# dist1ll/pomcpp

Hardware: AMD Instinct MI355X
Metric: env_steps_per_sec (higher is better)
Workload: dtype int32

## Files before the change

### pomcpp_amd/csrc/pom_step_body.h

```cpp
#ifndef POM_STEP_BODY_H_
#define POM_STEP_BODY_H_

#include "pom_packed.h"

#if defined(__clang__)
#define POM_NOUNROLL _Pragma("nounroll")
#else
#define POM_NOUNROLL
#endif
#define POM_N 11
#define POM_Q 20
#define POM_STACK_DEPTH 21

#if defined(POM_DIAG) && defined(__HIP_DEVICE_COMPILE__)
#define POM_STAMP(L, k)                                   \
    do {                                                  \
        const long long now_ = (long long)clock64();      \
        (L).t_acc[k] += now_ - (L).t_last;                \
        (L).t_last = now_;                                \
    } while (0)
#else
#define POM_STAMP(L, k) ((void)0)
#endif
#if defined(POM_TRUNC)
// ... 44 lines not shown
POM_HD int pb_pos(int b) { return b & 0xFF; }
POM_HD int pb_id(int b) { return (b >> 8) & 0xF; }
POM_HD int pb_strength(int b) { return (b >> 12) & 0xF; }
POM_HD int pb_time(int b) { return (b >> 16) & 0xF; }
POM_HD int pb_dir(int b) { return (b >> 20) & 0xF; }
POM_HD int pb_set(int b, uint32_t mask, uint32_t v) { return (int)(((uint32_t)b & ~mask) + v); }

#if defined(__HIP_DEVICE_COMPILE__)
#define POM_IN_VGPR(x) asm("" : "+v"(x))
#else
#define POM_IN_VGPR(x) ((void)0)
#endif
POM_HD int sel4(int i, const int v[4])
{
    int v0 = v[0], v1 = v[1], v2 = v[2], v3 = v[3];
    POM_IN_VGPR(v0);
    POM_IN_VGPR(v1);
    POM_IN_VGPR(v2);
    POM_IN_VGPR(v3);
    const int lo = (i & 1) ? v1 : v0, hi = (i & 1) ? v3 : v2;
    return (i & 2) ? hi : lo;
}
POM_HD uint32_t pick4(int i, const uint32_t v[4])
{
    const uint32_t lo = (i & 1) ? v[1] : v[0], hi = (i & 1) ? v[3] : v[2];
    return (i & 2) ? hi : lo;
}
POM_HD void put4(int i, int v[4], int x)
{
    v[0] = i == 0 ? x : v[0];
    v[1] = i == 1 ? x : v[1];
    v[2] = i == 2 ? x : v[2];
    v[3] = i == 3 ? x : v[3];
}
POM_HD int ag_x(int a0) { return a0 & 0xF; }
POM_HD int ag_y(int a0) { return (a0 >> 4) & 0xF; }
POM_HD int ag_pos(int a0) { return a0 & 0xFF; }
POM_HD int ag_dead(int a0) { return (a0 >> 17) & 1; }
POM_HD int ag_kick(int a0) { return (a0 >> 16) & 1; }
POM_HD int ag_setpos(int a0, int x, int y) { return (a0 & ~0xFF) | x | (y << 4); }
POM_HD int ag_bombcount(int a0) { return pom_sext8((uint32_t)a0 >> 8); }
POM_HD int ag_bombcount_add(int a0, int d) { return (a0 & ~0xFF00) | (int)(((uint32_t)a0 + ((uint32_t)d << 8)) & 0xFF00u); }
POM_HD int ag_max_bombs(int a1) { return pom_sext16((uint32_t)a1); }
POM_HD int ag_strength(int a1) { return (a1 >> 16) & 0xFF; }
POM_HD int ag_strength_inc(int a1) { return ag_strength(a1) == 0xFF ? a1 : a1 + (1 << 16); }

POM_HD int wrap20(int p)
{
    const unsigned u = (unsigned)p, w = u - (unsigned)POM_Q;
    return (int)(u < w ? u : w);
}
POM_HD uint32_t pom_zero_bytes(uint32_t x)
{
    return ~(((x & 0x7F7F7F7Fu) + 0x7F7F7F7Fu) | x | 0x7F7F7F7Fu);
}
POM_HD uint32_t pom_byte_x4(uint32_t b)
{
#if defined(__HIP_DEVICE_COMPILE__)
    return __builtin_amdgcn_perm(b, b, 0u);
#else
    return b * 0x01010101u;
#endif
}
template <int K>
POM_HD uint32_t pom_gather_bytes(uint32_t w0, uint32_t w1, uint32_t w2, uint32_t w3)
{
#if defined(__HIP_DEVICE_COMPILE__)
    const uint32_t lo = __builtin_amdgcn_perm(w1, w0, 0x0C0C0400u + K * 0x0101u);
    const uint32_t hi = __builtin_amdgcn_perm(w3, w2, 0x0C0C0400u + K * 0x0101u);
    return __builtin_amdgcn_perm(hi, lo, 0x05040100u);
#else
    return ((w0 >> (8 * K)) & 0xFFu) | (((w1 >> (8 * K)) & 0xFFu) << 8) | (((w2 >> (8 * K)) & 0xFFu) << 16) |
           (((w3 >> (8 * K)) & 0xFFu) << 24);
#endif
}
POM_HD int div11(int c)
{
#if defined(__HIP_DEVICE_COMPILE__)
    return __mul24(c, 373) >> 12;
#else
    return c / POM_N;
#endif
}
POM_HD int oob(int x, int y)
{
    const unsigned ux = (unsigned)x, uy = (unsigned)y;
    return (ux > uy ? ux : uy) >= (unsigned)POM_N;
}

POM_HD int mv_dx(int m) { return (int)((0x55555615u >> (2 * m)) & 3u) - 1; }
POM_HD int mv_dy(int m) { return (int)((0x55555561u >> (2 * m)) & 3u) - 1; }

template <class A>
struct PomStepper {
    A& a;
    PomLane& L;
    uint32_t oldp_ = 0;
    int irregular_ = 0;
    int folded_ = 0;
    uint32_t occ_[4] = {0u, 0u, 0u, 0u};
    int occ_valid_ = 0, occ_keep_ = 0;
    POM_HD PomStepper(A& a_, PomLane& l_) : a(a_), L(l_) {}

    POM_HD int bomb_at(int i) const { return a.bomb(wrap20(L.bIdx + i)); }
    POM_HD void set_bomb_at(int i, int v) { a.set_bomb(wrap20(L.bIdx + i), v); }

    POM_HD int bomb_index(int pos) const
    {
        int r = 99;
        POM_NOUNROLL
        for (int i = a.sub(); i < L.bCnt; i += A::G) {
            if (pb_pos(bomb_at(i)) == pos) {
                r = i;
                break;
            }
        }
        r = a.gmin(r);
        return r == 99 ? -1 : r;
    }
    POM_HD void put_bomb_at(int i, int v) { a.put_bomb(wrap20(L.bIdx + i), v); }
    POM_HD int bomb_index_alone(int pos) const
    {
        POM_NOUNROLL
        for (int i = 0; i < L.bCnt; i += 4) {
            const int b0 = bomb_at(i), b1 = bomb_at(i + 1), b2 = bomb_at(i + 2), b3 = bomb_at(i + 3);
            int r = -1;
            r = ((int)(i + 3 < L.bCnt) & (int)(pb_pos(b3) == pos)) ? i + 3 : r;
            r = ((int)(i + 2 < L.bCnt) & (int)(pb_pos(b2) == pos)) ? i + 2 : r;
            r = ((int)(i + 1 < L.bCnt) & (int)(pb_pos(b1) == pos)) ? i + 1 : r;
            r = pb_pos(b0) == pos ? i : r;
            if (r >= 0) return r;
        }
        return -1;
    }

    POM_HD int get_agent(int x, int y) const
    {
        const int want = x | (y << 4);
        int r = -1;
#pragma unroll
        for (int i = 3; i >= 0; i--)
            r = ((!ag_dead(L.a0[i])) & (int)(ag_pos(L.a0[i]) == want)) ? i : r;
        return r;
    }

    POM_HD void kill(int id)
    {
        if (id >= POM_AGENT_COUNT) {
            L.ub |= POM_UB_BAD_INDEX;
            return;
        }
        int v = sel4(id, L.a0);
        if (!ag_dead(v)) {
            put4(id, L.a0, v | POM_AG_DEAD);
            L.alive--;
        }
    }

    POM_HD void owner_bombcount_dec(int b)
    {
        int id = pb_id(b);
        if (id >= POM_AGENT_COUNT) {
            L.ub |= POM_UB_BAD_INDEX;
            return;
        }
        put4(id, L.a0, ag_bombcount_add(sel4(id, L.a0), -1));
    }

    POM_HD void remove_at(int at)
    {
        POM_NOUNROLL
        for (int i = at + 1 + a.sub(); i < L.bCnt; i += A::G) {
            const int v = bomb_at(i);
            put_bomb_at(i - 1, v);
        }
        a.sync();
        if (folded_) {
            const int w = bomb_at(L.bCnt - 1);
            set_bomb_at(L.bCnt - 1, (w & (1 << 24)) ? (w & ~(1 << 24)) : (int)((uint32_t)w + (1u << 16)));
        }
        L.bCnt--;
    }

    enum { REM_TOP = 62, REM_NONE = 63 };

    POM_HD int owner_strength(int b)
    {
        const int owner = pb_id(b);
        if (owner < POM_AGENT_COUNT) return ag_strength(a.ag1(owner));
        L.ub |= POM_UB_BAD_INDEX;
        return 0;
    }

    POM_HD void flame_prologue(int x, int y, int strength, int e )
    {
        int slot = L.fIdx + L.fCnt;
        if (__builtin_expect(slot >= 2 * POM_Q, 0)) {
            POM_NOUNROLL
            while (slot >= POM_Q) slot -= POM_Q;
        } else {
            slot = wrap20(slot);
        }
        a.set_flame(slot, x | (y << 8) | (POM_FLAME_LIFETIME << 16) | ((strength & 0xFF) << 24));
        if (__builtin_expect(L.fCnt >= 255, 0)) L.ub |= POM_UB_FLAME_QUEUE_RANGE;
        else L.fCnt++;
        const int c = y * POM_N + x;
        if (pc_is_agent(e)) kill(pc_agent_id(e));
        a.set_cell(c, POM_C_FLAME + c);
    }
    POM_HD void flame_prologue(int x, int y, int strength) { flame_prologue(x, y, strength, a.cell(y * POM_N + x)); }

    POM_HD void explode_epilogue(int rem)
    {
        if (rem == REM_TOP) {
            owner_bombcount_dec(bomb_at(0));
            L.bIdx = wrap20(L.bIdx + 1);
            L.bCnt--;
        } else if (rem != REM_NONE) {
            owner_bombcount_dec(bomb_at(rem));
            remove_at(rem);
        }
    }

    POM_HD static int ray_step(int dir)
    {
        return (int)(int8_t)(0xF50BFF01u >> (8 * dir));
    }
    POM_HD static int ray_cell(int c0, int dir, int i)
    {
#if defined(__HIP_DEVICE_COMPILE__)
        return c0 + __mul24(i, ray_step(dir));
#else
        return c0 + i * ray_step(dir);
#endif
    }
    POM_HD static int ray_room(int x, int y, int s, int dir)
    {
        const unsigned rooms = (unsigned)(POM_N - 1 - x) | ((unsigned)x << 4) | ((unsigned)(POM_N - 1 - y) << 8) | ((unsigned)y << 12);
        const int room = (int)((rooms >> (4 * dir)) & 0xFu);
        return room < s ? room : s;
    }

    POM_HD void kill_set(int victims)
    {
#pragma unroll
        for (int j = 0; j < 4; j++) {
            const int hit = (victims >> j) & 1 & !ag_dead(L.a0[j]);
            L.a0[j] |= hit << 17;
            L.alive -= hit;
        }
    }

    POM_HD void explode(int x, int y, int strength, int rem, int top_word = -1)
    {
        int s = strength < 0 ? 0 : strength > POM_N ? POM_N : strength;
        POM_STAMP(L, POM_PH_TICK_BOMBS);
        if (s > 2) {
            explode_long(x, y, strength, rem);
            return;
        }
        {
            const int c0 = y * POM_N + x;
            const int e0 = a.cell(c0);
            int chains = 0, victims = 0;
            int chain_key = 0;
            uint32_t lens = 0;
            uint32_t ends = 0;
            POM_NOUNROLL
            for (int r = a.sub(); r < 4; r += A::G) {
                const int lim = ray_room(x, y, s, r);
                const int on1 = lim >= 1, on2 = lim >= 2;
                const int c1 = ray_cell(c0, r, on1);
                const int e1 = a.cell(c1);
                const int ag1 = pc_is_agent(e1);
                int q1 = 0;
                if (on1 & ((int)(e1 == POM_C_BOMB) | ag1)) {
                    const int cy = div11(c1);
                    q1 = bomb_index_alone((c1 - cy * POM_N) | (cy << 4)) >= 0;
                }
                const int took1 = on1 & !q1 & (int)(e1 != POM_C_RIGID);
                const int wood1 = took1 & pc_is_wood(e1);
                int len = took1, vict = (took1 & ag1) << (pc_agent_id(e1) & 3), flag = wood1 ? pc_wood_flag(e1) : 0;
                if (q1) {
                    chains = 1;
                    chain_key = (1 << 12) | ag1 | ((pc_agent_id(e1) & 3) << 1);
                }
                if (took1 & !wood1 & on2) {
                    const int c2 = ray_cell(c0, r, 2);
                    const int e2 = a.cell(c2);
                    const int ag2 = pc_is_agent(e2);
                    int q2 = 0;
                    if ((int)(e2 == POM_C_BOMB) | ag2) {
                        const int cy = div11(c2);
                        q2 = bomb_index_alone((c2 - cy * POM_N) | (cy << 4)) >= 0;
                    }
                    const int took2 = (int)(q2 == 0) & (int)(e2 != POM_C_RIGID);
                    len += took2;
                    vict |= (took2 & ag2) << (pc_agent_id(e2) & 3);
                    flag = (took2 & pc_is_wood(e2)) ? pc_wood_flag(e2) : flag;
                    if (q2) {
                        chains = 1;
                        chain_key = (2 << 12) | ag2 | ((pc_agent_id(e2) & 3) << 1);
                    }
                }
                victims |= vict;
                ends |= (uint32_t)flag << (2 * r);
                lens |= (uint32_t)len << (4 * r);
            }
            if (__builtin_expect(!a.gor(chains), 1)) {
                flame_prologue(x, y, strength, e0);
                const int killed = a.gor(victims);
                if (killed) kill_set(killed);
                POM_NOUNROLL
                for (int r = a.sub(); r < 4; r += A::G) {
                    const int len = (lens >> (4 * r)) & 0xF, f = (int)((ends >> (2 * r)) & 3u);
                    if (len >= 1) a.put_cell(ray_cell(c0, r, 1), pc_flame_code(c0, r, 1, len == 1 ? f : 0));
                    if (len >= 2) a.put_cell(ray_cell(c0, r, 2), pc_flame_code(c0, r, 2, f));
                }
                a.sync();
                if (rem == REM_TOP && top_word != -1) {
                    owner_bombcount_dec(top_word);
                    L.bIdx = wrap20(L.bIdx + 1);
                    L.bCnt--;
                } else {
                    explode_epilogue(rem);
                }
                return;
            }
            if (A::G == 4) {
                const int r = a.sub();
                explode_long(x, y, strength, rem, 1, (int)((lens >> (4 * r)) & 0xF), (int)((ends >> (2 * r)) & 3u), victims, chain_key, e0);
                return;
            }
        }
        explode_long(x, y, strength, rem);
    }

    POM_HD void bomb_cells(uint32_t occ[4]) const
    {
        occ[0] = occ[1] = occ[2] = occ[3] = 0u;
        if (A::G == 1) {
            POM_NOUNROLL
            for (int k = 0; k < L.bCnt; k++) {
                const int b = bomb_at(k);
                const int idx = pb_y(b) * POM_N + pb_x(b);
// ... 39 lines not shown
        int r = 99;
#pragma unroll
        for (int q = NS - 1; q >= 0; q--) {
            const int k = a.sub() + q * A::G;
            r = (k < L.bCnt && pb_pos(w[q]) == pos) ? k : r;
        }
        r = a.gmin(r);
        return r == 99 ? -1 : r;
    }

    POM_HD void scan_ray(int c0, int r, int start, int lim, const uint32_t occ[4], int& len, int& ends, int& wood, int& vict, int& chain,
                         int& info)
    {
        constexpr int W = 4;
        len = start - 1;
        ends = wood = vict = chain = info = 0;
        const uint32_t H = 0x80808080u;
        POM_NOUNROLL
        for (int i0 = start; i0 <= lim; i0 += W) {
            uint32_t d = 0;
#pragma unroll
            for (int q = 0; q < W; q++)
                d |= (uint32_t)a.cell(ray_cell(c0, r, i0 + q <= lim ? i0 + q : lim)) << (8 * q);
            const int n = lim - i0 + 1;
            const uint32_t onray = n >= W ? H : H >> (8 * (W - n));
            const uint32_t l = d & 0x7F7F7F7Fu, lo = ~d;
            const uint32_t ge1 = l + 0x7F7F7F7Fu, ge2 = l + 0x7E7E7E7Eu, ge3 = l + 0x7D7D7D7Du, ge6 = l + 0x7A7A7A7Au, ge11 = l + 0x75757575u,
                           ge15 = l + 0x71717171u;
            const uint32_t rigid = ge1 & ~ge2 & lo, bombc = ge2 & ~ge3 & lo, woodc = ge6 & ~ge11 & lo & onray, agentc = ge11 & ~ge15 & lo & H;
            const uint32_t fixed = ((rigid | woodc) & onray & H) | (~onray & H);
            const uint32_t fixed_low = fixed & (0u - fixed);
            uint32_t cand = (bombc | agentc) & H & (fixed_low - 1u);
            uint32_t chain_at = 0u;
            POM_NOUNROLL
            while (cand) {
                const int q = __builtin_ctz(cand) >> 3;
                if (cell_in(occ, ray_cell(c0, r, i0 + q))) {
                    chain_at = cand & (0u - cand);
                    break;
                }
                cand &= cand - 1u;
            }
            const uint32_t stop = fixed | chain_at;
            const uint32_t at = stop & (0u - stop), below = at - 1u;
            const int before = __builtin_popcount(below & H);
            const int on_wood = (at & woodc) != 0u;
            len = i0 - 1 + before + on_wood;
            uint32_t dead = agentc & below;
            POM_NOUNROLL
            while (dead) {
                const int q = __builtin_ctz(dead) >> 3;
                dead &= dead - 1u;
                vict |= 1 << pc_agent_id((int)((d >> (8 * q)) & 0xFFu));
            }
            if (at) {
                const int e = (int)((d >> (8 * before)) & 0xFFu);
                if (on_wood) {
                    ends = pc_wood_flag(e);
                    wood = 1;
                }
                if (at & chain_at) {
                    chain = i0 + before;
                    info = pc_is_agent(e) | ((pc_agent_id(e) & 3) << 1);
                }
                break;
            }
        }
    }

    POM_HD void explode_long(int x, int y, int strength, int rem, int seen = 0, int seen_len = 0, int seen_ends = 0, int seen_vict = 0,
                             int seen_chain = 0, int seen_origin = 0)
    {
        int s = strength < 0 ? 0 : strength > POM_N ? POM_N : strength;
        POM_STAMP(L, POM_PH_TICK_BOMBS);
        if (seen) flame_prologue(x, y, strength, seen_origin);
        else flame_prologue(x, y, strength);
        int dir = 0, i = 1, sp = 0;
        constexpr int NR = 4 / A::G;
        uint32_t (&occ)[4] = occ_;
        if (!occ_valid_) bomb_cells(occ);
        occ_valid_ = occ_keep_;
        POM_NOUNROLL
        for (;;) {
            const int c0 = y * POM_N + x;
            int first = 0x7FFFFFFF;
            int rstar, jq = -1;
            if (A::G == 1) {
                POM_NOUNROLL
                for (int r = dir; r < 4 && first == 0x7FFFFFFF; r++) {
                    const int rs1 = r == dir ? i : 1;
                    int len1, ends1, wood1, vict1, chain1, info1;
                    scan_ray(c0, r, rs1, ray_room(x, y, s, r), occ, len1, ends1, wood1, vict1, chain1, info1);
                    if (chain1) {
                        const int c = ray_cell(c0, r, chain1);
                        const int cy = div11(c);
                        jq = bomb_index((c - cy * POM_N) | (cy << 4));
                        if (jq < 0) {
                            const uint32_t m = ~(1u << (c & 31));
                            const int w = c >> 5;
                            occ[0] &= w == 0 ? m : ~0u; occ[1] &= w == 1 ? m : ~0u; occ[2] &= w == 2 ? m : ~0u; occ[3] &= w == 3 ? m : ~0u;
                            r--;
                            continue;
                        }
                        first = (r << 16) | (chain1 << 12) | info1;
                    }
                    POM_NOUNROLL
                    for (int d = rs1; d <= len1; d++)
                        a.put_cell(ray_cell(c0, r, d), pc_flame_code(c0, r, d, (wood1 && d == len1) ? ends1 : 0));
                    kill_set(vict1);
                }
                rstar = first == 0x7FFFFFFF ? 4 : first >> 16;
            } else {
            int rs[NR], rlen[NR], rends[NR], rwood[NR], rvict[NR];
#pragma unroll
            for (int q = 0; q < NR; q++) {
                const int r = a.sub() + q * A::G;
                rs[q] = r == dir ? i : 1;
                int chain = 0, info = 0;
                rlen[q] = rs[q] - 1;
                rends[q] = rwood[q] = rvict[q] = 0;
                if (seen) {
                    rlen[q] = seen_len;
                    rends[q] = seen_ends;
                    rwood[q] = 1;
                    rvict[q] = seen_vict;
                    chain = seen_chain >> 12;
                    info = seen_chain & 0xFFF;
                } else if (r >= dir) scan_ray(c0, r, rs[q], ray_room(x, y, s, r), occ, rlen[q], rends[q], rwood[q], rvict[q], chain, info);
                const int key = (r << 16) | (chain << 12) | info;
                first = (chain != 0 && key < first) ? key : first;
            }
            first = a.gmin(first);
            seen = 0;
            rstar = first == 0x7FFFFFFF ? 4 : first >> 16;
            if (rstar < 4) {
                const int c = ray_cell(c0, rstar, (first >> 12) & 0xF);
                const int cy = div11(c);
                jq = bomb_index_wide((c - cy * POM_N) | (cy << 4));
                if (jq < 0) {
                    const uint32_t m = ~(1u << (c & 31));
                    const int w = c >> 5;
                    occ[0] &= w == 0 ? m : ~0u; occ[1] &= w == 1 ? m : ~0u; occ[2] &= w == 2 ? m : ~0u; occ[3] &= w == 3 ? m : ~0u;
                    continue;
                }
            }
            POM_STAMP(L, POM_PH_X_SCAN);
            int victims = 0;
#pragma unroll
            for (int q = 0; q < NR; q++) {
                const int r = a.sub() + q * A::G;
                if (r >= dir && r <= rstar) {
                    victims |= rvict[q];
                    POM_NOUNROLL
                    for (int d = rs[q]; d <= rlen[q]; d++)
                        a.put_cell(ray_cell(c0, r, d), pc_flame_code(c0, r, d, (rwood[q] && d == rlen[q]) ? rends[q] : 0));
                }
            }
            {
                const int killed = a.gor(victims);
                if (killed) kill_set(killed);
            }
            }
            POM_STAMP(L, POM_PH_X_COMMIT);
            if (rstar == 4) {
                explode_epilogue(rem);
                POM_STAMP(L, POM_PH_X_EPILOGUE);
                if (sp == 0) return;
                sp--;
                const int fr = a.frame(sp);
                x = fr & 0xF; y = (fr >> 4) & 0xF; s = (fr >> 8) & 0xF;
                dir = (fr >> 12) & 7; i = (fr >> 15) & 0xF; rem = (fr >> 19) & 63;
                const int pc0 = y * POM_N + x;
                const int c = ray_cell(pc0, dir, i);
                const int e = a.cell(c);
                int go_on = 0;
                if (e != POM_C_RIGID) {
                    const int was_wood = pc_is_wood(e);
                    a.set_cell(c, pc_flame_code(pc0, dir, i, was_wood ? pc_wood_flag(e) : 0));
                    go_on = !was_wood;
                }
                if (go_on) i++;
                else { dir++; i = 1; }
                continue;
            }
            const int d = (first >> 12) & 0xF;
            if (first & 1) kill((first >> 1) & 3);
            if (sp >= POM_STACK_DEPTH) {
                L.ub |= POM_UB_BAD_INDEX;
                return;
            }
            a.set_frame(sp, x | (y << 4) | (s << 8) | (rstar << 12) | (d << 15) | (rem << 19));
            sp++;
            const int st2 = owner_strength(bomb_at(jq));
            const int c = ray_cell(c0, rstar, d);
            y = div11(c);
            x = c - y * POM_N;
            rem = jq;
            flame_prologue(x, y, st2);
            s = st2 < 0 ? 0 : st2 > POM_N ? POM_N : st2;
            dir = 0;
            i = 1;
            POM_STAMP(L, POM_PH_X_NEST);
        }
    }

    POM_HD void flames_dec(int& top, int& n)
    {
        top = 0;
        n = L.fCnt;
        if (L.fCnt <= 0) return;
        int p = L.fIdx + a.sub();
        p = wrap20(p);
        int held_any = 0;
        POM_NOUNROLL
        for (int i = a.sub(); i < L.fCnt; i += A::G) {
            const int f = a.flame(p);
            const int held = (f & 0xFF0000) == 0x800000;
            const int nf = held ? f : (f & ~0xFF0000) | ((f - 0x10000) & 0xFF0000);
            held_any |= held;
            a.put_flame(p, nf);
            if (p == L.fIdx) top = nf;
            p = wrap20(p + A::G);
        }
        const int v = a.gor(top | (held_any << 7));
        top = v & ~0x80;
        if (v & 0x80) L.ub |= POM_UB_FLAME_QUEUE_RANGE;
    }
    POM_HD void flame_pops(int top, int n)
    {
        POM_NOUNROLL
        for (int k = 0; k < n; k++) {
            const int f = k == 0 ? top : a.flame(L.fIdx);
            if (((f >> 16) & 0xFF) != 0) break;
            const int x = f & 0xFF, y = (f >> 8) & 0xFF;
            int s = (f >> 24) & 0xFF;
            s = s > POM_N ? POM_N : s;
            if (!oob(x, y)) {
                const int c0 = y * POM_N + x;
                if (a.cell(c0) == POM_C_FLAME + c0) a.set_cell(c0, POM_C_PASSAGE);
                POM_NOUNROLL
                for (int r = a.sub(); r < 4; r += A::G) {
                    const int lim = ray_room(x, y, s, r);
                    {
                        const int c = ray_cell(c0, r, lim >= 1);
                        const int to = pc_flame_pops_to(a.cell(c), c0, r, 1);
                        if ((int)(lim >= 1) & (int)(to >= 0)) a.put_cell(c, to);
                    }
                    POM_NOUNROLL
                    for (int i = 2; i <= lim; i++) {
                        const int c = ray_cell(c0, r, i);
                        const int to = pc_flame_pops_to(a.cell(c), c0, r, i);
                        if (to >= 0) a.put_cell(c, to);
                    }
                }
            }
            L.fIdx = wrap20(L.fIdx + 1);
            L.fCnt--;
        }
    }

    POM_HD void chain_reversion(uint32_t mvp, int id, int bombs_move = 1)
    {
        POM_NOUNROLL
        for (int hop = 0;; hop++) {
            if (hop >= 8) {
                L.ub |= POM_UB_REVERT_LOOP;
                return;
            }
            const int av = sel4(id, L.a0);
            const int m = (mvp >> (4 * id)) & 0xF;
            const int ox = ag_x(av) - mv_dx(m), oy = ag_y(av) - mv_dy(m);
            if (oob(ox, oy)) return;
            const int origin_agent = get_agent(ox, oy);
            const int okey = (ox + 1) | ((oy + 1) << 4);
            int bd = -1;
            if (bombs_move) {
                bd = 99;
                POM_NOUNROLL
                for (int i = a.sub(); i < L.bCnt; i += A::G) {
                    if (a.bdest(i) == okey) {
                        bd = i;
                        break;
                    }
                }
                bd = a.gmin(bd);
                if (bd == 99) bd = -1;
            }
            put4(id, L.a0, ag_setpos(av, ox, oy));
            irregular_ |= (ox | (oy << 4)) != (int)((oldp_ >> (8 * id)) & 0xFF);
            a.set_cell(oy * POM_N + ox, POM_C_AGENT + id);
            if (origin_agent != -1) {
                id = origin_agent;
                continue;
            }
            if (bd != -1) {
                const int b = bomb_at(bd);
                const int dir = pb_dir(b);
                if (mv_dx(dir) == 0 && mv_dy(dir) == 0) {
                    a.set_cell(oy * POM_N + ox, POM_C_AGENT + id);
                    return;
                }
                const int bx = ox - mv_dx(dir), by = oy - mv_dy(dir);
                if (oob(bx, by)) {
                    L.ub |= POM_UB_BAD_INDEX;
                    return;
                }
                const int has_agent = get_agent(bx, by);
                set_bomb_at(bd, pb_set(pb_set(b, 0xF00000u, 0), 0xFFu, (uint32_t)bx + ((uint32_t)by << 4)));
                a.set_cell(by * POM_N + bx, POM_C_BOMB);
                if (has_agent != -1) {
                    id = has_agent;
                    continue;
                }
            }
            return;
        }
    }

    POM_HD int bomb_target_key(int b) const
    {
        const int d = pb_dir(b);
        return (pb_x(b) + mv_dx(d) + 1) | ((pb_y(b) + mv_dy(d) + 1) << 4);
    }

    POM_HD int bomb_collision(uint32_t mvp, int k)
    {
        const int b = bomb_at(k);
        const int key = bomb_target_key(b);
// ... 12 lines not shown
            set_bomb_at(k, nb);
            const int ag = get_agent(pb_x(nb), pb_y(nb));
            if (ag > -1) {
                const int m = (mvp >> (4 * ag)) & 0xF;
                if (m != POM_MOVE_IDLE && m != POM_MOVE_BOMB) {
                    unforeseen_ = 1;
                    chain_reversion(mvp, ag);
                    const int cur = bomb_at(k);
                    a.set_cell(pb_y(cur) * POM_N + pb_x(cur), POM_C_BOMB);
                }
            }
        }
        return collided;
    }

    POM_HD void loop_a_bomb(int mvp, int oldp, int k, int bombs_move)
    {
        const int b = bomb_at(k);
        const int bx = pb_x(b), by = pb_y(b), d = pb_dir(b);
        const int tx = bx + mv_dx(d), ty = by + mv_dy(d);
        int blocked = oob(tx, ty);
        if (!blocked) {
            const int e = a.cell(ty * POM_N + tx);
            blocked = pc_blocks_bomb(e);
        }
        if (blocked) {
            set_bomb_at(k, pb_set(b, 0xF00000u, 0));
            const int ag = get_agent(bx, by);
            if (ag > -1) {
                const int m = (mvp >> (4 * ag)) & 0xF;
                const int av = sel4(ag, L.a0);
                const int was = (oldp >> (8 * ag)) & 0xFF;
                if ((int)(m != POM_MOVE_IDLE) & (int)(m != POM_MOVE_BOMB) & (int)((ag_x(av) | (ag_y(av) << 4)) != was)) {
                    chain_reversion(mvp, ag, bombs_move);
                    if (get_agent(bx, by) == -1) a.set_cell(by * POM_N + bx, POM_C_BOMB);
                }
            }
        }
    }

    POM_HD void step(const int mv_in[4]) { step_packed(pack_moves(mv_in)); }
    POM_HD static int clamp_move(int m) { return ((unsigned)m <= 5u) ? m : 6; }
    POM_HD static uint32_t pack_moves(const int mv_in[4])
    {
        uint32_t mvp = 0;
#pragma unroll
        for (int i = 0; i < 4; i++) mvp |= (uint32_t)clamp_move(mv_in[i]) << (4 * i);
        return mvp;
    }
    POM_HD uint32_t pack_moves_quad(int mine) const
    {
        const int c = clamp_move(mine);
        return (uint32_t)a.template gbcast<0>(c) | ((uint32_t)a.template gbcast<1>(c) << 4) | ((uint32_t)a.template gbcast<2>(c) << 8) |
               ((uint32_t)a.template gbcast<3>(c) << 12);
    }
    POM_HD void step_packed(uint32_t mvp)
    {
        int ftop, fn, btop, bn;
        flames_dec(ftop, fn);
        POM_STAMP(L, POM_PH_FLAMES_DEC);
        POM_CUT(L, 10);
        flame_pops(ftop, fn);
        POM_STAMP(L, POM_PH_FLAMES);
        POM_CUT(L, 20);
        step_middle(mvp, btop, bn);
        top_explosions(btop, bn);
        POM_STAMP(L, POM_PH_TICK_BOMBS);
    }
    POM_HD void top_explosions(int top, int n)
    {
        occ_valid_ = 0;
        occ_keep_ = 1;
        POM_NOUNROLL
        for (int k = 0; k < n && L.bCnt > 0; k++) {
            const int c = k == 0 ? top : bomb_at(0);
            if (pb_time(c) != 0) break;
            explode(pb_x(c), pb_y(c), pb_strength(c), REM_TOP, c);
        }
        occ_valid_ = occ_keep_ = 0;
    }
    POM_HD void prep_positions(const uint32_t mvp, uint32_t& oldp, uint32_t& dstp, int& deadmask, int& contact, int& clash)
    {
        oldp = dstp = 0;
        deadmask = 0;
#pragma unroll
        for (int i = 0; i < 4; i++) deadmask |= ag_dead(L.a0[i]) << i;
        contact = 0;
        clash = 0;
        if (A::G == 4) {
            const int m = a.sub();
            const int av = sel4(m, L.a0);
            const int mvm = (int)((mvp >> (4 * m)) & 0xF);
            const int pxm = ag_x(av), pym = ag_y(av);
            const int dxm = pxm + mv_dx(mvm), dym = pym + mv_dy(mvm);
            const int pos8 = ag_pos(av);
            oldp = (uint32_t)a.template gbcast<0>(pos8) | ((uint32_t)a.template gbcast<1>(pos8) << 8) |
                   ((uint32_t)a.template gbcast<2>(pos8) << 16) | ((uint32_t)a.template gbcast<3>(pos8) << 24);
            const int d8 = ((dxm + 1) & 0xF) | (((dym + 1) & 0xF) << 4);
            dstp = (uint32_t)a.template gbcast<0>(d8) | ((uint32_t)a.template gbcast<1>(d8) << 8) |
                   ((uint32_t)a.template gbcast<2>(d8) << 16) | ((uint32_t)a.template gbcast<3>(d8) << 24);
            const uint32_t want = (uint32_t)((dxm & 0xF) | ((dym & 0xF) << 4));
            const uint32_t others = ~(0x80u << (8 * m));
            const uint32_t dead80 = (((uint32_t)deadmask * 0x00204081u) & 0x01010101u) << 7;
            const uint32_t hit_d = pom_zero_bytes(oldp ^ (want * 0x01010101u)) & others;
            const uint32_t hit_p = pom_zero_bytes(oldp ^ ((uint32_t)pos8 * 0x01010101u)) & others & ~dead80;
            int mine = (int)(hit_d != 0u) | ((int)((hit_p != 0u) & !ag_dead(av)) << 1);
            mine = a.gor(mine);
            contact = mine & 1;
            clash = mine >> 1;
        } else {
#pragma unroll
            for (int i = 0; i < 4; i++) {
                const int px = ag_x(L.a0[i]), py = ag_y(L.a0[i]);
                const int mvi = (int)((mvp >> (4 * i)) & 0xF);
                const int dx = px + mv_dx(mvi), dy = py + mv_dy(mvi);
                oldp |= (uint32_t)(px | (py << 4)) << (8 * i);
                dstp |= (uint32_t)(((dx + 1) & 0xF) | (((dy + 1) & 0xF) << 4)) << (8 * i);
            }
#pragma unroll
            for (int i = 0; i < 4; i++)
#pragma unroll
                for (int j = 0; j < 4; j++)
                    if (i != j) contact |= ((((dstp >> (8 * i)) & 0xF) - 1) & 0xF) == ((oldp >> (8 * j)) & 0xF) &&
                                           ((((dstp >> (8 * i + 4)) & 0xF) - 1) & 0xF) == ((oldp >> (8 * j + 4)) & 0xF);
        }
    }
    POM_HD void prep_dependencies(const uint32_t mvp, const uint32_t oldp, const int deadmask, uint32_t& dstp, uint32_t& dep, uint32_t& roots,
                                  int& nroots)
    {
        int px[4], py[4], dx[4], dy[4];
#pragma unroll
        for (int i = 0; i < 4; i++) {
            px[i] = (int)((oldp >> (8 * i)) & 0xF);
            py[i] = (int)((oldp >> (8 * i + 4)) & 0xF);
            const int mvi = (int)((mvp >> (4 * i)) & 0xF);
            dx[i] = px[i] + mv_dx(mvi);
            dy[i] = py[i] + mv_dy(mvi);
        }
        roots = 0xFFFF;
        nroots = 0;
#pragma unroll
        for (int i = 0; i < 4; i++) {
#pragma unroll
            for (int j = i; j < 4; j++) {
                if ((int)(dx[i] == px[j]) & (int)(dy[i] == py[j]) & (int)(dx[j] == px[i]) & (int)(dy[j] == py[i])) {
                    dx[i] = px[i]; dy[i] = py[i];
                    dx[j] = px[j]; dy[j] = py[j];
                }
            }
        }
#pragma unroll
        for (int i = 0; i < 4; i++) {
            int is_root = 1;
            if (!((deadmask >> i) & 1)) {
#pragma unroll
                for (int j = 0; j < 4; j++) {
                    if (j == i) continue;
                    if (is_root & !((deadmask >> j) & 1) & (int)(dx[i] == px[j]) & (int)(dy[i] == py[j])) {
                        dep = (dep & ~(0xFu << (4 * j))) | ((uint32_t)i << (4 * j));
                        is_root = 0;
                    }
                }
            }
            if (is_root) {
                roots = (roots & ~(0xFu << (4 * nroots))) | ((uint32_t)i << (4 * nroots));
                nroots++;
            }
        }
        dstp = 0;
#pragma unroll
        for (int i = 0; i < 4; i++) dstp |= (uint32_t)(((dx[i] + 1) & 0xF) | (((dy[i] + 1) & 0xF) << 4)) << (8 * i);
    }

    int unforeseen_ = 0;
    POM_HD uint32_t loop_b_todo()
    {
        a.claims_clear();
        a.sync();
        POM_NOUNROLL
        for (int k = a.sub(); k < L.bCnt; k += A::G) {
            const int b = bomb_at(k);
            const int d = pb_dir(b);
            const int bx = pb_x(b), by = pb_y(b), tx = bx + mv_dx(d), ty = by + mv_dy(d);
            a.claim(by * POM_N + bx);
            if ((int)(d != 0) & !oob(tx, ty) & (int)((mv_dx(d) | mv_dy(d)) != 0)) a.claim(ty * POM_N + tx);
        }
        a.sync();
        uint32_t f = 0;
// ... 33 lines not shown
            }
            if (bomb_collision(mvp, k)) return;
            b = bomb_at(k);
            set_bomb_at(k, pb_set(b, 0xFFu, (uint32_t)tx + ((uint32_t)ty << 4)));
            if (bomb_index(bx | (by << 4)) < 0 && a.cell(by * POM_N + bx) == POM_C_BOMB)
                a.set_cell(by * POM_N + bx, POM_C_PASSAGE);
            te = a.cell(tc);
            if (pc_is_walkable(te)) a.set_cell(tc, POM_C_BOMB);
            if (!pc_is_flame(te)) return;
        }
        const int j = bomb_index(tx | (ty << 4));
        const int jb = bomb_at(j);
        unforeseen_ = 1;
        explode(pb_x(jb), pb_y(jb), owner_strength(jb), j);
    }

    POM_HD void step_middle(const uint32_t mvp, int& top, int& n)
    {
        top = 0;
        n = 0;

        uint32_t oldp = 0, dstp = 0;
        uint32_t dep = 0xFFFF, roots = 0x3210;
        int nroots = 4;
        int deadmask = 0, contact = 0, clash = 0;
        prep_positions(mvp, oldp, dstp, deadmask, contact, clash);
        oldp_ = oldp;
        POM_CUT(L, 24);
        if (contact) prep_dependencies(mvp, oldp, deadmask, dstp, dep, roots, nroots);
        POM_CUT(L, 27);
        const int ouroboros = nroots == 0;
        int posb[4];
#pragma unroll
        for (int i = 0; i < 4; i++) posb[i] = (int)((oldp >> (8 * i)) & 0xFF);

        int on_bomb = 0;
        POM_NOUNROLL
        for (int k = a.sub(); k < L.bCnt; k += A::G) {
            const int bw = bomb_at(k);
            const int bp = pb_pos(bw);
#pragma unroll
            for (int j = 0; j < 4; j++) on_bomb |= (bp == posb[j]) << j;
            on_bomb |= (pb_dir(bw) != 0) << 4;
        }
        on_bomb = a.gor(on_bomb);
        POM_STAMP(L, POM_PH_AGENT_PREP);
        POM_CUT(L, 30);
        int agents_done = 0;
        if (A::G == 4) {
            int par = !ouroboros && !clash;
            uint32_t rankp = 0x3210u, depthp = 0u;
            int rounds = 1;
            if (par && nroots != 4) {
                const int ri = a.sub();
                int i = ri < nroots ? (int)((roots >> (4 * ri)) & 0xF) : 0xF;
                uint32_t dp = 0u, memb = 0u;
                int len = 0;
#pragma unroll
                for (int d = 0; d < 4; d++) {
                    const int on = i != 0xF;
                    const int sh = 4 * (i & 3);
                    dp |= on ? (uint32_t)d << sh : 0u;
                    memb |= on ? 0xFu << sh : 0u;
                    len += on;
                    i = on ? (int)((dep >> sh) & 0xF) : 0xF;
                }
                const int l0 = a.template gbcast<0>(len), l1 = a.template gbcast<1>(len), l2 = a.template gbcast<2>(len),
                          l3 = a.template gbcast<3>(len);
                const int b_lo = (ri & 1) ? l0 : 0, b_hi = (ri & 1) ? l0 + l1 + l2 : l0 + l1;
                const int base = (ri & 2) ? b_hi : b_lo;
                rankp = (uint32_t)a.gor((int)((dp + (uint32_t)base * 0x1111u) & memb));
                depthp = (uint32_t)a.gor((int)dp);
                par = l0 + l1 + l2 + l3 == 4;
                const int m01 = l0 > l1 ? l0 : l1, m23 = l2 > l3 ? l2 : l3;
                rounds = m01 > m23 ? m01 : m23;
            }
            if (par) {
                agents_done = 1;
                const int m = a.sub();
                int av = sel4(m, L.a0), a1v = a.ag1(m);
                const int a1_before = a1v;
                const int mvm = (mvp >> (4 * m)) & 0xF;
                const int live = !ag_dead(av);
                const int myrank = (int)((rankp >> (4 * m)) & 0xF), mydepth = (int)((depthp >> (4 * m)) & 0xF);
                const int wants = live & (int)(mvm == POM_MOVE_BOMB) & (int)(ag_bombcount(av) < ag_max_bombs(a1v));
                const uint32_t w_all = (uint32_t)a.gor(wants << (4 * m + 3));
                const uint32_t not_before = (rankp | 0x8888u) - (uint32_t)myrank * 0x1111u;
                const int slot_off = __builtin_popcount(w_all & ~not_before);
                const int fits = wants & (int)(L.bCnt + slot_off < POM_Q);
                int ubm = (wants & !fits) ? POM_UB_QUEUE_OVERFLOW : 0;
                int planted_moving = 0;
                if (fits) {
                    const int slot = wrap20(L.bIdx + L.bCnt + slot_off);
                    int b = a.bomb(slot);
                    planted_moving = pb_dir(b) != 0;
                    b = pb_set(b, 0xF00u, (uint32_t)m << 8);
                    b = pb_set(b, 0xFFu, (uint32_t)ag_x(av) + ((uint32_t)ag_y(av) << 4));
                    b = pb_set(b, 0xF000u, (uint32_t)ag_strength(a1v) << 12);
                    b = pb_set(b, 0xF0000u, (uint32_t)(POM_BOMB_LIFETIME + 1) << 16);
                    a.put_bomb(slot, b);
                    av = ag_bombcount_add(av, 1);
                }
                const int walks = live & (int)(mvm != POM_MOVE_IDLE) & (int)(mvm != POM_MOVE_BOMB);
                const int x = ag_x(av), y = ag_y(av);
                const int dkey = (dstp >> (8 * m)) & 0xFF;
                const int ddx = (dkey & 0xF) - 1, ddy = (dkey >> 4) - 1;
                const int goes = walks & !oob(ddx, ddy);
                const int dc = ddy * POM_N + ddx, oc = y * POM_N + x;
                const int vacated = ((on_bomb >> m) & 1) ? POM_C_BOMB : POM_C_PASSAGE;
                const uint32_t same_dest = pom_zero_bytes(dstp ^ pom_byte_x4((uint32_t)dkey)) & ~(0x80u << (8 * m));
                uint32_t dead80 = (((uint32_t)deadmask * 0x00204081u) & 0x01010101u) << 7;
                const int dread = goes ? dc : oc;
                const int dpos = (ddx | (ddy << 4)) & 0xFF;
                int died_sum = 0;
                const int still_moving = (int)(nroots != 4) | ((on_bomb >> 4) & 1);
                POM_NOUNROLL
                for (int r = 0; r < rounds; r++) {
                    const int act = goes & (int)(mydepth == r);
                    const int item = a.cell(dread);
                    const int shows_me = a.cell(oc) == POM_C_AGENT + m;
                    const int collide = (same_dest & ~dead80) != 0u;
                    const int flame = pc_is_flame(item), pu = pc_is_powerup(item);
                    const int died = act & flame;
                    const int free_way = act & !flame & !collide;
                    const int to_passage = free_way & (pu | (int)(item == POM_C_PASSAGE));
                    const int to_bomb = free_way & (int)(item == POM_C_BOMB);
                    const int kicker = ag_kick(av);
                    const int bombs_move = a.gor((to_bomb & kicker) | planted_moving | still_moving) & 1;
                    if (to_passage & pu) {
                        a1v = item == POM_C_EXTRABOMB ? (a1v & ~0xFFFF) | ((a1v + 1) & 0xFFFF) : a1v;
                        a1v = item == POM_C_INCRRANGE ? ag_strength_inc(a1v) : a1v;
                        av |= (int)(item == POM_C_KICK) << 16;
                    }
                    int bounce = 0;
                    if (to_bomb & (kicker | ((int)(bombs_move == 0) & shows_me))) {
                        const int bi = bomb_index_alone(dpos);
                        const int found = bi >= 0;
                        if (kicker & found) put_bomb_at(bi, pb_set(bomb_at(bi), 0xF00000u, (uint32_t)mvm << 20));
                        ubm |= (kicker & !found) ? POM_UB_NULL_BOMB : 0;
                        bounce = (int)(kicker == 0) & found;
                    }
                    const int steps_on = to_bomb & !bounce;
                    const int moves = to_passage | steps_on;
                    if (((died | to_passage) & shows_me) | steps_on) a.put_cell(oc, vacated);
                    if (moves) a.put_cell(dc, POM_C_AGENT + m);
                    av = moves ? (av & ~0xFF) | dpos : av;
                    av |= died << 17;
                    died_sum += died;
                    if (r + 1 < rounds) dead80 |= (uint32_t)a.gor(died << (8 * m + 7));
                }
                L.a0[0] = a.template gbcast<0>(av); L.a0[1] = a.template gbcast<1>(av);
                L.a0[2] = a.template gbcast<2>(av); L.a0[3] = a.template gbcast<3>(av);
                if (a1v != a1_before) a.put_ag1(m, a1v);
                L.alive -= a.gadd(died_sum);
                L.bCnt += a.gadd(fits);
                L.ub |= (uint32_t)a.gor(ubm);
            }
        }
        if (!agents_done) {
            int root_idx = 0;
            int i = ouroboros ? 0 : (int)(roots & 0xF);
            POM_NOUNROLL
            for (int n = 0; n < 4; n++) {
                if (i == 0xF) {
                    root_idx++;
                    const int nx = root_idx < 4 ? (int)((roots >> (4 * root_idx)) & 0xF) : 0xF;
                    if (nx == 0xF) {
                        L.ub |= POM_UB_LOST_AGENT;
                        break;
                    }
                    i = nx;
                }
                const int m = (mvp >> (4 * i)) & 0xF;
                const int av = sel4(i, L.a0);
                const int next = (int)((dep >> (4 * i)) & 0xF);
                if (ag_dead(av) || m == POM_MOVE_IDLE) {
                    i = next;
                    continue;
                }
                const int x = ag_x(av), y = ag_y(av);
                if (m == POM_MOVE_BOMB) {
                    const int a1v = a.ag1(i);
                    const int bomb_count = ag_bombcount(av), max_bombs = ag_max_bombs(a1v);
                    if (bomb_count < max_bombs) {
                        if (L.bCnt >= POM_Q) {
                            L.ub |= POM_UB_QUEUE_OVERFLOW;
                        } else {
                            const int slot = wrap20(L.bIdx + L.bCnt);
                            int b = a.bomb(slot);
                            b = pb_set(b, 0xF00u, (uint32_t)i << 8);
                            b = pb_set(b, 0xFFu, (uint32_t)x + ((uint32_t)y << 4));
                            b = pb_set(b, 0xF000u, (uint32_t)ag_strength(a1v) << 12);
                            b = pb_set(b, 0xF0000u, (uint32_t)(POM_BOMB_LIFETIME + 1) << 16);
                            a.set_bomb(slot, b);
                            put4(i, L.a0, ag_bombcount_add(av, 1));
                            L.bCnt++;
#pragma unroll
                            for (int j = 0; j < 4; j++) on_bomb |= (ag_pos(L.a0[j]) == ag_pos(av)) << j;
                        }
                    }
                    i = next;
                    continue;
                }
                const int dkey = (dstp >> (8 * i)) & 0xFF;
                const int ddx = (dkey & 0xF) - 1, ddy = (dkey >> 4) - 1;
                if (oob(ddx, ddy)) {
                    i = next;
                    continue;
                }
                const int dc = ddy * POM_N + ddx;
                int item = a.cell(dc);
                if (ouroboros && bomb_index(ddx | (ddy << 4)) >= 0) item = POM_C_BOMB;

                if (pc_is_flame(item)) {
                    kill(i);
                    deadmask |= 1 << i;
                    const int oc = y * POM_N + x;
                    if (a.cell(oc) == POM_C_AGENT + i)
                        a.set_cell(oc, ((on_bomb >> i) & 1) ? POM_C_BOMB : POM_C_PASSAGE);
                    i = next;
                    continue;
                }
                int collide = 0;
#pragma unroll
                for (int j = 0; j < 4; j++)
                    collide |= (j != i) & !((deadmask >> j) & 1) & (((dstp >> (8 * j)) & 0xFF) == (uint32_t)dkey);
                if (collide) {
                    i = next;
                    continue;
                }
                if (pc_is_powerup(item)) {
                    if (item == POM_C_EXTRABOMB) {
                        const int a1v = a.ag1(i);
                        a.set_ag1(i, (a1v & ~0xFFFF) | ((a1v + 1) & 0xFFFF));
                    } else if (item == POM_C_INCRRANGE) {
                        a.set_ag1(i, ag_strength_inc(a.ag1(i)));
                    } else {
                        put4(i, L.a0, sel4(i, L.a0) | POM_AG_KICK);
                    }
                    item = POM_C_PASSAGE;
                }
                const int oc = y * POM_N + x;
                if (item == POM_C_PASSAGE || (ouroboros && pc_is_agent(item))) {
                    if (a.cell(oc) == POM_C_AGENT + i)
                        a.set_cell(oc, ((on_bomb >> i) & 1) ? POM_C_BOMB : POM_C_PASSAGE);
                    a.set_cell(dc, POM_C_AGENT + i);
                    put4(i, L.a0, ag_setpos(sel4(i, L.a0), ddx, ddy));
                } else if (item == POM_C_BOMB) {
                    a.set_cell(oc, ((on_bomb >> i) & 1) ? POM_C_BOMB : POM_C_PASSAGE);
                    a.set_cell(dc, POM_C_AGENT + i);
                    const int cur = sel4(i, L.a0);
                    put4(i, L.a0, ag_setpos(cur, ddx, ddy));
                    if (ag_kick(cur)) {
                        const int bi = bomb_index(ddx | (ddy << 4));
                        if (bi < 0) L.ub |= POM_UB_NULL_BOMB;
                        else set_bomb_at(bi, pb_set(bomb_at(bi), 0xF00000u, (uint32_t)m << 20));
                    }
                }
                i = next;
            }
        }

        POM_STAMP(L, POM_PH_AGENT_LOOP);
        POM_CUT(L, 40);
        if (L.bCnt > 0) {
            int moving = 0;
            int ripe = 0;
            uint32_t cand = 0;
            int late = 0;
            uint32_t movers = 0;
            const uint32_t nowp = pom_gather_bytes<0>((uint32_t)L.a0[0], (uint32_t)L.a0[1], (uint32_t)L.a0[2], (uint32_t)L.a0[3]);
            const uint32_t nowflags = pom_gather_bytes<2>((uint32_t)L.a0[0], (uint32_t)L.a0[1], (uint32_t)L.a0[2], (uint32_t)L.a0[3]);
            const uint32_t nowdead80 = (nowflags << 6) & 0x80808080u;
            POM_NOUNROLL
            for (int k = a.sub(); k < L.bCnt; k += A::G) {
                int b = pb_set(bomb_at(k), 0xF000000u, 0);
                const int key = bomb_target_key(b);
                if (pb_time(b) == 0) {
                    late = 1;
                    b |= 1 << 24;
                } else {
                    b = (int)((uint32_t)b - (1u << 16));
                }
                put_bomb_at(k, b);
                if (k == 0) top = b;
                a.put_bdest(k, key);
                moving |= pb_dir(b) != 0;
                movers |= (uint32_t)(pb_dir(b) != 0) << k;
                const int idx = pb_y(b) * POM_N + pb_x(b);
                if (idx < POM_CELLS) {
                    const int e = a.cell(idx);
                    ripe |= (e == POM_C_PASSAGE) | pc_is_flame(e);
                    const uint32_t hit = pom_zero_bytes(nowp ^ pom_byte_x4((uint32_t)pb_pos(b))) & ~nowdead80;
                    const int sh = __builtin_ctz(hit | 0x80000000u) - 7;
                    const int m2 = (mvp >> (sh >> 1)) & 0xF;
                    const int was = (oldp >> sh) & 0xFF;
                    cand |= (uint32_t)(pc_blocks_bomb(e) & (int)(hit != 0u) & (int)(m2 != POM_MOVE_IDLE) & (int)(m2 != POM_MOVE_BOMB) &
                                       (int)(pb_pos(b) != was)) << k;
                }
            }
            if (A::G > 1) {
                const uint32_t fl = (uint32_t)a.gor((int)(cand | ((uint32_t)ripe << 20) | ((uint32_t)late << 21) | ((uint32_t)moving << 23)));
                cand = fl & 0xFFFFFu;
                ripe = (int)((fl >> 20) & 1u);
                late = (int)((fl >> 21) & 1u);
                moving = (int)((fl >> 23) & 1u);
                movers = (uint32_t)a.gor((int)movers);
            }
            folded_ = 1;
            int touched = cand != 0;
            POM_STAMP(L, POM_PH_BOMB_PASS);
            POM_CUT(L, 50);
            int next = 0;
            {
                uint32_t todo = cand | movers;
                irregular_ = 0;
                POM_NOUNROLL
                while (todo && !irregular_) {
                    const int k = __builtin_ctz(todo);
                    todo &= todo - 1u;
                    loop_a_bomb(mvp, oldp, k, moving);
                    next = k + 1;
                }
                if (!irregular_) next = L.bCnt;
            }
            POM_NOUNROLL
            for (int k = next; k < L.bCnt; k++) loop_a_bomb(mvp, oldp, k, moving);
            POM_STAMP(L, POM_PH_BOMB_A);
            POM_CUT(L, 60);
            touched |= moving | ripe;
            int general = moving;
            if (!general && ripe) {
                int in_flame = 0;
                POM_NOUNROLL
                for (int k = a.sub(); k < L.bCnt; k += A::G) {
                    const int b = bomb_at(k);
                    in_flame |= pc_is_flame(a.cell(pb_y(b) * POM_N + pb_x(b)));
                }
                if (!a.gor(in_flame)) {
                    POM_NOUNROLL
                    for (int k = a.sub(); k < L.bCnt; k += A::G) {
                        const int b = bomb_at(k);
                        const int c = pb_y(b) * POM_N + pb_x(b);
                        if (a.cell(c) == POM_C_PASSAGE) a.put_cell(c, POM_C_BOMB);
                    }
                } else {
                    general = 1;
                }
            }
            if (general) {
                uint32_t todo = loop_b_todo();
                POM_NOUNROLL
                while (todo) {
                    const int k = __builtin_ctz(todo);
                    todo &= todo - 1u;
                    if (k >= L.bCnt) break;
                    unforeseen_ = 0;
                    loop_b_bomb(mvp, k);
                    if (unforeseen_) todo = k + 1 < POM_Q ? ((1u << POM_Q) - 1u) & ~((2u << k) - 1u) : 0u;
                }
            }
            POM_STAMP(L, POM_PH_BOMB_B);
            POM_CUT(L, 70);
            if (late) {
                POM_NOUNROLL
                for (int k = a.sub(); k < L.bCnt; k += A::G) {
                    const int b = bomb_at(k);
                    if (b & (1 << 24)) put_bomb_at(k, (int)(((uint32_t)b & ~(1u << 24)) - (1u << 16)));
                }
                touched = 1;
            }
            folded_ = 0;
// ... 41 lines not shown
```

Baseline: 9.459 billion.

## Hoist cell reads, gather positions bytewise, and use mul24 cell indexing

Adds a pom_cell helper that uses __mul24 for cell indexing, and builds oldp with a byte-permute gather instead of four broadcasts. Dead-agent bits are now computed once from L.a0 and cached in a member. In the agent move loop, the destination and own-cell reads are issued before the bomb-placement section and reloaded only between rounds. In flame decay, the first ray's cell is loaded together with the centre cell. The aim is to cut cross-lane broadcasts, integer multiply cost and load latency on the step path. The changes are several small micro-optimizations, each guarded by a disable macro; hoisting the reads above bomb placement could change semantics if placement writes those cells.

```diff
diff --git a/pomcpp_amd/csrc/pom_step_body.h b/pomcpp_amd/csrc/pom_step_body.h
--- a/pomcpp_amd/csrc/pom_step_body.h
+++ b/pomcpp_amd/csrc/pom_step_body.h
@@ -150,6 +150,18 @@
     return c / POM_N;
 #endif
 }
+POM_HD int pom_cell(int x, int y)
+{
+#if defined(__HIP_DEVICE_COMPILE__) && !defined(POM_NO_MULTIPASS)
+    return __mul24(y, POM_N) + x;
+#else
+    return y * POM_N + x;
+#endif
+}
+POM_HD uint32_t pom_dead80(const int a0[4])
+{
+    return (pom_gather_bytes<2>((uint32_t)a0[0], (uint32_t)a0[1], (uint32_t)a0[2], (uint32_t)a0[3]) << 6) & 0x80808080u;
+}
 POM_HD int oob(int x, int y)
 {
     const unsigned ux = (unsigned)x, uy = (unsigned)y;
@@ -164,6 +176,7 @@
     A& a;
     PomLane& L;
     uint32_t oldp_ = 0;
+    uint32_t dead80_ = 0;
     int irregular_ = 0;
     int folded_ = 0;
     uint32_t occ_[4] = {0u, 0u, 0u, 0u};
@@ -272,11 +285,11 @@
         a.set_flame(slot, x | (y << 8) | (POM_FLAME_LIFETIME << 16) | ((strength & 0xFF) << 24));
         if (__builtin_expect(L.fCnt >= 255, 0)) L.ub |= POM_UB_FLAME_QUEUE_RANGE;
         else L.fCnt++;
-        const int c = y * POM_N + x;
+        const int c = pom_cell(x, y);
         if (pc_is_agent(e)) kill(pc_agent_id(e));
         a.set_cell(c, POM_C_FLAME + c);
     }
-    POM_HD void flame_prologue(int x, int y, int strength) { flame_prologue(x, y, strength, a.cell(y * POM_N + x)); }
+    POM_HD void flame_prologue(int x, int y, int strength) { flame_prologue(x, y, strength, a.cell(pom_cell(x, y))); }
 
     POM_HD void explode_epilogue(int rem)
     {
@@ -328,7 +341,7 @@
             return;
         }
         {
-            const int c0 = y * POM_N + x;
+            const int c0 = pom_cell(x, y);
             const int e0 = a.cell(c0);
             int chains = 0, victims = 0;
             int chain_key = 0;
@@ -534,7 +547,7 @@
         occ_valid_ = occ_keep_;
         POM_NOUNROLL
         for (;;) {
-            const int c0 = y * POM_N + x;
+            const int c0 = pom_cell(x, y);
             int first = 0x7FFFFFFF;
             int rstar, jq = -1;
             if (A::G == 1) {
@@ -622,7 +635,7 @@
                 const int fr = a.frame(sp);
                 x = fr & 0xF; y = (fr >> 4) & 0xF; s = (fr >> 8) & 0xF;
                 dir = (fr >> 12) & 7; i = (fr >> 15) & 0xF; rem = (fr >> 19) & 63;
-                const int pc0 = y * POM_N + x;
+                const int pc0 = pom_cell(x, y);
                 const int c = ray_cell(pc0, dir, i);
                 const int e = a.cell(c);
                 int go_on = 0;
@@ -688,14 +701,25 @@
             int s = (f >> 24) & 0xFF;
             s = s > POM_N ? POM_N : s;
             if (!oob(x, y)) {
-                const int c0 = y * POM_N + x;
+                const int c0 = pom_cell(x, y);
+#if !defined(POM_NO_POPS_BATCH)
+                const int centre = a.cell(c0);
+                const int e_first = a.cell(ray_cell(c0, a.sub(), ray_room(x, y, s, a.sub()) >= 1));
+                if (centre == POM_C_FLAME + c0) a.set_cell(c0, POM_C_PASSAGE);
+#else
                 if (a.cell(c0) == POM_C_FLAME + c0) a.set_cell(c0, POM_C_PASSAGE);
+#endif
                 POM_NOUNROLL
                 for (int r = a.sub(); r < 4; r += A::G) {
                     const int lim = ray_room(x, y, s, r);
                     {
                         const int c = ray_cell(c0, r, lim >= 1);
-                        const int to = pc_flame_pops_to(a.cell(c), c0, r, 1);
+#if !defined(POM_NO_POPS_BATCH)
+                        const int e = r == a.sub() ? e_first : a.cell(c);
+#else
+                        const int e = a.cell(c);
+#endif
+                        const int to = pc_flame_pops_to(e, c0, r, 1);
                         if ((int)(lim >= 1) & (int)(to >= 0)) a.put_cell(c, to);
                     }
                     POM_NOUNROLL
@@ -874,6 +898,7 @@
     POM_HD void prep_positions(const uint32_t mvp, uint32_t& oldp, uint32_t& dstp, int& deadmask, int& contact, int& clash)
     {
         oldp = dstp = 0;
+        dead80_ = 0;
         deadmask = 0;
 #pragma unroll
         for (int i = 0; i < 4; i++) deadmask |= ag_dead(L.a0[i]) << i;
@@ -886,16 +911,26 @@
             const int pxm = ag_x(av), pym = ag_y(av);
             const int dxm = pxm + mv_dx(mvm), dym = pym + mv_dy(mvm);
             const int pos8 = ag_pos(av);
+#if !defined(POM_NO_PREP_GATHER)
+            oldp = pom_gather_bytes<0>((uint32_t)L.a0[0], (uint32_t)L.a0[1], (uint32_t)L.a0[2], (uint32_t)L.a0[3]);
+#else
             oldp = (uint32_t)a.template gbcast<0>(pos8) | ((uint32_t)a.template gbcast<1>(pos8) << 8) |
                    ((uint32_t)a.template gbcast<2>(pos8) << 16) | ((uint32_t)a.template gbcast<3>(pos8) << 24);
+#endif
             const int d8 = ((dxm + 1) & 0xF) | (((dym + 1) & 0xF) << 4);
             dstp = (uint32_t)a.template gbcast<0>(d8) | ((uint32_t)a.template gbcast<1>(d8) << 8) |
                    ((uint32_t)a.template gbcast<2>(d8) << 16) | ((uint32_t)a.template gbcast<3>(d8) << 24);
             const uint32_t want = (uint32_t)((dxm & 0xF) | ((dym & 0xF) << 4));
             const uint32_t others = ~(0x80u << (8 * m));
-            const uint32_t dead80 = (((uint32_t)deadmask * 0x00204081u) & 0x01010101u) << 7;
+#if !defined(POM_NO_MULTIPASS)
+            const uint32_t dead80 = dead80_ = pom_dead80(L.a0);
+            const uint32_t hit_d = pom_zero_bytes(oldp ^ pom_byte_x4(want)) & others;
+            const uint32_t hit_p = pom_zero_bytes(oldp ^ pom_byte_x4((uint32_t)pos8)) & others & ~dead80;
+#else
+            const uint32_t dead80 = dead80_ = (((uint32_t)deadmask * 0x00204081u) & 0x01010101u) << 7;
             const uint32_t hit_d = pom_zero_bytes(oldp ^ (want * 0x01010101u)) & others;
             const uint32_t hit_p = pom_zero_bytes(oldp ^ ((uint32_t)pos8 * 0x01010101u)) & others & ~dead80;
+#endif
             int mine = (int)(hit_d != 0u) | ((int)((hit_p != 0u) & !ag_dead(av)) << 1);
             mine = a.gor(mine);
             contact = mine & 1;
@@ -1095,6 +1130,16 @@
                 const int a1_before = a1v;
                 const int mvm = (mvp >> (4 * m)) & 0xF;
                 const int live = !ag_dead(av);
+                const int walks = live & (int)(mvm != POM_MOVE_IDLE) & (int)(mvm != POM_MOVE_BOMB);
+                const int x = ag_x(av), y = ag_y(av);
+                const int dkey = (dstp >> (8 * m)) & 0xFF;
+                const int ddx = (dkey & 0xF) - 1, ddy = (dkey >> 4) - 1;
+                const int goes = walks & !oob(ddx, ddy);
+                const int dc = pom_cell(ddx, ddy), oc = pom_cell(x, y);
+                const int dread = goes ? dc : oc;
+#if !defined(POM_NO_ROUND_HOIST)
+                int item_now = a.cell(dread), own_now = a.cell(oc);
+#endif
                 const int myrank = (int)((rankp >> (4 * m)) & 0xF), mydepth = (int)((depthp >> (4 * m)) & 0xF);
                 const int wants = live & (int)(mvm == POM_MOVE_BOMB) & (int)(ag_bombcount(av) < ag_max_bombs(a1v));
                 const uint32_t w_all = (uint32_t)a.gor(wants << (4 * m + 3));
@@ -1114,24 +1159,22 @@
                     a.put_bomb(slot, b);
                     av = ag_bombcount_add(av, 1);
                 }
-                const int walks = live & (int)(mvm != POM_MOVE_IDLE) & (int)(mvm != POM_MOVE_BOMB);
-                const int x = ag_x(av), y = ag_y(av);
-                const int dkey = (dstp >> (8 * m)) & 0xFF;
-                const int ddx = (dkey & 0xF) - 1, ddy = (dkey >> 4) - 1;
-                const int goes = walks & !oob(ddx, ddy);
-                const int dc = ddy * POM_N + ddx, oc = y * POM_N + x;
                 const int vacated = ((on_bomb >> m) & 1) ? POM_C_BOMB : POM_C_PASSAGE;
                 const uint32_t same_dest = pom_zero_bytes(dstp ^ pom_byte_x4((uint32_t)dkey)) & ~(0x80u << (8 * m));
-                uint32_t dead80 = (((uint32_t)deadmask * 0x00204081u) & 0x01010101u) << 7;
-                const int dread = goes ? dc : oc;
+                uint32_t dead80 = dead80_;
                 const int dpos = (ddx | (ddy << 4)) & 0xFF;
                 int died_sum = 0;
                 const int still_moving = (int)(nroots != 4) | ((on_bomb >> 4) & 1);
                 POM_NOUNROLL
                 for (int r = 0; r < rounds; r++) {
                     const int act = goes & (int)(mydepth == r);
+#if !defined(POM_NO_ROUND_HOIST)
+                    const int item = item_now;
+                    const int shows_me = own_now == POM_C_AGENT + m;
+#else
                     const int item = a.cell(dread);
                     const int shows_me = a.cell(oc) == POM_C_AGENT + m;
+#endif
                     const int collide = (same_dest & ~dead80) != 0u;
                     const int flame = pc_is_flame(item), pu = pc_is_powerup(item);
                     const int died = act & flame;
@@ -1160,7 +1203,13 @@
                     av = moves ? (av & ~0xFF) | dpos : av;
                     av |= died << 17;
                     died_sum += died;
-                    if (r + 1 < rounds) dead80 |= (uint32_t)a.gor(died << (8 * m + 7));
+                    if (r + 1 < rounds) {
+                        dead80 |= (uint32_t)a.gor(died << (8 * m + 7));
+#if !defined(POM_NO_ROUND_HOIST)
+                        item_now = a.cell(dread);
+                        own_now = a.cell(oc);
+#endif
+                    }
                 }
                 L.a0[0] = a.template gbcast<0>(av); L.a0[1] = a.template gbcast<1>(av);
                 L.a0[2] = a.template gbcast<2>(av); L.a0[3] = a.template gbcast<3>(av);
@@ -1300,7 +1349,7 @@
                 a.put_bdest(k, key);
                 moving |= pb_dir(b) != 0;
                 movers |= (uint32_t)(pb_dir(b) != 0) << k;
-                const int idx = pb_y(b) * POM_N + pb_x(b);
+                const int idx = pom_cell(pb_x(b), pb_y(b));
                 if (idx < POM_CELLS) {
                     const int e = a.cell(idx);
                     ripe |= (e == POM_C_PASSAGE) | pc_is_flame(e);
```

Result: no change. 9.390 billion (-0.7%).
